# mobvoi/lstm_ctc

Measured on AMD Instinct MI355X. Metric: acoustic frames/sec (whole node), 5xBiLSTM-1024 CTC, higher is better.
Workload: dtype f32

## Files before the change

### include/lstm_ctc_hip.h

```cpp
#ifndef LSTM_CTC_HIP_H
#define LSTM_CTC_HIP_H

#include <stddef.h>
#include <stdint.h>

#ifdef __cplusplus
extern "C" {
#endif

#define LC_OK 0
#define LC_EINVAL (-1)
#define LC_ELAUNCH (-2)
#define LC_EWORKSPACE (-3)

typedef void *lc_stream_t;

const char *lc_last_error(void);
int lc_version(void);

#define LC_OPTION_UNSET (-0x7fffffffL - 1)
int lc_set_option(const char *name, long value);
int lc_get_option(const char *name, long *value);

size_t lc_ctc_workspace_bytes(int T, int B, int V, int max_label_len);
// ... 109 lines not shown
size_t lc_optimizer_workspace_bytes(size_t n);

size_t lc_colsum_workspace_bytes(int N);
int lc_colsum(const float *x, int rows, int N, int ldx, float *out, int accumulate, void *workspace,
              size_t workspace_bytes, lc_stream_t stream);
int lc_transpose(const float *in, int rows, int cols, float *out, lc_stream_t stream);

int lc_label_smoothing(const float *logits, int rows, int V, const float *log_q, float weight,
                       double *loss_acc, float *dlogits, lc_stream_t stream);

int lc_posteriors(const float *logits, int rows, int V, float smooth, int apply_softmax,
                  int apply_log, const float *log_prior, float *out, lc_stream_t stream);

size_t lc_bn_workspace_bytes(int C);
int lc_bn_moments(const float *x, int rows, int C, int ldx, float *mean, float *var, void *workspace,
                  size_t workspace_bytes, lc_stream_t stream);
int lc_bn_apply(const float *x, int rows, int C, int ldx, const float *mean, const float *var,
                const float *gamma, const float *beta, float eps, float *y, int ldy, lc_stream_t stream);
int lc_bn_bwd(const float *x, const float *dy, int rows, int C, int ldx, int lddy, const float *mean,
              const float *var, const float *gamma, float eps, int training, float *dx, int lddx,
              float *dgamma, float *dbeta, void *workspace, size_t workspace_bytes, lc_stream_t stream);
int lc_bn_update_moving(float *moving_mean, float *moving_var, const float *mean, const float *var, int C,
                        float momentum, lc_stream_t stream);
int lc_length_mask(float *x, int T, int B, int C, int ldx, const int *seq_len, lc_stream_t stream);

int lc_pack_rows(const float *x, int ldx, const int *rows, int Mp, int C, float *out, int ldo, lc_stream_t stream);
int lc_unpack_rows(const float *x, int ldx, const int *inverse, int rows, int C, float *out, int ldo, lc_stream_t stream);

void lc_debug_set_lstm_stamps(unsigned long long *buf);
int lc_debug_last_lstm_schedule(void);
void lc_debug_set_ctc_stamps(unsigned long long *buf);
int lc_debug_spin(int blocks, int microseconds, int lds_bytes, lc_stream_t stream);
int lc_debug_gemm_whole_round_row_tiles(int row_tiles, int col_tiles, int cus);

typedef struct {
    int64_t num_frames;
    int32_t dim;
    int32_t has_input, has_target;
    int64_t num_labels;
} lc_seqex_info_t;
int lc_tfrecord_inspect(const void *file, size_t nbytes, int verify_crc, lc_seqex_info_t *info);
int lc_tfrecord_decode(const void *file, size_t nbytes, int dim, int left_context, int right_context, int subsample,
                       float *x, size_t x_row_stride, int64_t max_rows, int64_t *labels, int64_t max_labels);
uint32_t lc_crc32c(const void *data, size_t nbytes);
typedef struct lc_batch_reader lc_batch_reader_t;
int lc_batch_open(const char *const *paths, int n, int verify_crc, int expect_dim, int nthreads,
                  lc_batch_reader_t **reader, int64_t *num_frames, int64_t *num_labels);
int lc_batch_decode(lc_batch_reader_t *reader, int left_context, int right_context, int subsample, float *x,
                    size_t utt_stride, size_t row_stride, int64_t max_rows, int64_t *labels, size_t label_stride,
                    int64_t max_labels, int64_t pad_label, int nthreads);
void lc_batch_close(lc_batch_reader_t *reader);

#ifdef __cplusplus
}
#endif
#endif
```

### lstm_ctc_amd/_lib.py

```python
import ctypes
import os

_HERE = os.path.dirname(os.path.abspath(__file__))
LIB_PATH = os.path.join(_HERE, "liblstm_ctc_hip.so")

c_int, c_float, c_void_p, c_size_t = ctypes.c_int, ctypes.c_float, ctypes.c_void_p, ctypes.c_size_t
c_u32 = ctypes.c_uint32

SIGNATURES = {
    "lc_last_error": (ctypes.c_char_p, []),
    "lc_version": (c_int, []),
    "lc_set_option": (c_int, [ctypes.c_char_p, ctypes.c_long]),
    "lc_get_option": (c_int, [ctypes.c_char_p, ctypes.POINTER(ctypes.c_long)]),
    "lc_ctc_workspace_bytes": (c_size_t, [c_int, c_int, c_int, c_int]),
    "lc_ctc_loss": (c_int, [c_void_p, c_int, c_int, c_int, c_void_p, c_void_p, c_void_p, c_int, c_void_p,
                            c_void_p, c_void_p, c_size_t, c_void_p]),
    "lc_ctc_greedy": (c_int, [c_void_p, c_int, c_int, c_int, c_void_p, c_void_p, c_void_p, c_void_p, c_void_p]),
    "lc_edit_distance_host": (c_int, [c_void_p, c_int, c_void_p, c_void_p, c_void_p, c_int, c_void_p]),
    "lc_gemm_workspace_bytes": (c_size_t, [c_int, c_int, c_int]),
    "lc_gemm_f32": (c_int, [c_int, c_int, c_int, c_int, c_int, c_float, c_void_p, c_int, c_void_p, c_int,
                            c_float, c_void_p, c_int, c_void_p, c_void_p, c_size_t, c_void_p]),
    "lc_gemm_bf16": (c_int, [c_int, c_int, c_int, c_int, c_int, c_float, c_void_p, c_int, c_void_p, c_int,
                             c_float, c_void_p, c_int, c_void_p, c_void_p, c_size_t, c_void_p]),
    "lc_bn_workspace_bytes": (c_size_t, [c_int]),
# ... 21 lines not shown
                                  c_void_p, c_void_p, ctypes.c_size_t, c_void_p]),
    "lc_gemm_next_epilogue": (c_int, [c_void_p]),
    "lc_gemm_bf16_nn": (c_int, [c_int, c_int, c_int, c_float, c_void_p, c_int, c_void_p, c_int, c_float, c_void_p, c_int,
                                c_void_p, c_void_p, c_size_t, c_void_p]),
    "lc_debug_set_lstm_stamps": (None, [c_void_p]),
    "lc_debug_set_ctc_stamps": (None, [c_void_p]),
    "lc_debug_spin": (c_int, [c_int, c_int, c_int, c_void_p]),
    "lc_length_mask": (c_int, [c_void_p, c_int, c_int, c_int, c_int, c_void_p, c_void_p]),
    "lc_pack_rows": (c_int, [c_void_p, c_int, c_void_p, c_int, c_int, c_void_p, c_int, c_void_p]),
    "lc_unpack_rows": (c_int, [c_void_p, c_int, c_void_p, c_int, c_int, c_void_p, c_int, c_void_p]),
    "lc_lstm_fwd_workspace_bytes": (c_size_t, [c_int, c_int, c_int]),
    "lc_lstm_fwd": (c_int, [c_void_p, c_int, c_void_p, c_int, c_int, c_int, c_float, c_void_p, c_size_t, c_void_p]),
    "lc_lstm_fwd_bf16": (c_int, [c_void_p, c_int, c_void_p, c_int, c_int, c_int, c_float, c_void_p, c_size_t, c_void_p]),
    "lc_lstm_fwd_x3": (c_int, [c_void_p, c_int, c_void_p, c_int, c_int, c_int, c_float, c_void_p, c_size_t, c_void_p]),
    "lc_lstm_bwd_x3": (c_int, [c_void_p, c_int, c_void_p, c_int, c_int, c_int, c_void_p, c_size_t, c_void_p]),
    "lc_lstm_bwd_workspace_bytes": (c_size_t, [c_int, c_int, c_int]),
    "lc_lstm_bwd_bf16": (c_int, [c_void_p, c_int, c_void_p, c_int, c_int, c_int, c_void_p, c_size_t, c_void_p]),
    "lc_lstm_bwd": (c_int, [c_void_p, c_int, c_void_p, c_int, c_int, c_int, c_void_p, c_size_t, c_void_p]),
    "lc_dropout_scale": (c_int, [c_void_p, c_int, c_int, c_int, c_float, c_u32, c_u32, c_void_p, c_int, c_int,
                                 c_void_p]),
    "lc_dropout_scale_bf16": (c_int, [c_void_p, c_int, c_int, c_int, c_float, c_u32, c_u32, c_void_p, c_int, c_int,
                                      c_void_p, c_int, c_void_p]),
    "lc_moe_combine_fwd": (c_int, [c_void_p, c_void_p, c_int, c_int, c_int, c_float, c_float, c_u32, c_void_p,
                                   c_void_p, c_void_p]),
    "lc_moe_combine_bwd": (c_int, [c_void_p, c_void_p, c_void_p, c_int, c_int, c_int, c_float, c_float, c_u32,
                                   c_void_p, c_void_p]),
    "lc_optimizer_workspace_bytes": (c_size_t, [c_size_t]),
    "lc_optimizer_step": (c_int, [c_void_p, c_void_p, c_size_t, c_size_t, c_float, c_float, c_int, c_float,
                                  c_int, c_void_p, c_void_p, c_void_p, c_void_p, c_size_t, c_void_p]),
    "lc_colsum_workspace_bytes": (c_size_t, [c_int]),
    "lc_colsum": (c_int, [c_void_p, c_int, c_int, c_int, c_void_p, c_int, c_void_p, c_size_t, c_void_p]),
    "lc_debug_last_lstm_schedule": (c_int, []),
    "lc_debug_gemm_whole_round_row_tiles": (c_int, [c_int, c_int, c_int]),
    "lc_transpose": (c_int, [c_void_p, c_int, c_int, c_void_p, c_void_p]),
    "lc_label_smoothing": (c_int, [c_void_p, c_int, c_int, c_void_p, c_float, c_void_p, c_void_p, c_void_p]),
    "lc_tfrecord_inspect": (c_int, [c_void_p, c_size_t, c_int, c_void_p]),
    "lc_tfrecord_decode": (c_int, [c_void_p, c_size_t, c_int, c_int, c_int, c_int, c_void_p, c_size_t, ctypes.c_int64,
                                   c_void_p, ctypes.c_int64]),
    "lc_crc32c": (c_u32, [c_void_p, c_size_t]),
    "lc_batch_open": (c_int, [c_void_p, c_int, c_int, c_int, c_int, c_void_p, c_void_p, c_void_p]),
    "lc_batch_decode": (c_int, [c_void_p, c_int, c_int, c_int, c_void_p, c_size_t, c_size_t, ctypes.c_int64, c_void_p,
                                c_size_t, ctypes.c_int64, ctypes.c_int64, c_int]),
    "lc_batch_close": (None, [c_void_p]),
    "lc_posteriors": (c_int, [c_void_p, c_int, c_int, c_float, c_int, c_int, c_void_p, c_void_p, c_void_p]),
}


class GemmEpilogue(ctypes.Structure):
    _fields_ = [("keep", ctypes.c_float), ("seed", ctypes.c_uint32), ("stream0", ctypes.c_uint32),
                ("drop_width", ctypes.c_int), ("c_bf16", ctypes.c_void_p), ("ldc_bf16", ctypes.c_int),
                ("shadow_only", ctypes.c_int)]


class SeqExInfo(ctypes.Structure):
    _fields_ = [("num_frames", ctypes.c_int64), ("dim", ctypes.c_int32), ("has_input", ctypes.c_int32),
                ("has_target", ctypes.c_int32), ("num_labels", ctypes.c_int64)]


class LstmFwdDir(ctypes.Structure):
    _fields_ = [("zx", c_void_p), ("R", c_void_p), ("w_f", c_void_p), ("w_i", c_void_p), ("w_o", c_void_p),
                ("cs", c_void_p), ("hs", c_void_p), ("reverse", c_int), ("hs_bf16", c_void_p), ("shadow_only", c_int)]


class LstmBwdDir(ctypes.Structure):
    _fields_ = [("gates", c_void_p), ("RT", c_void_p), ("w_f", c_void_p), ("w_i", c_void_p), ("w_o", c_void_p),
                ("cs", c_void_p), ("dh", c_void_p), ("dpeep", c_void_p), ("dbias", c_void_p), ("reverse", c_int),
# ... 39 lines not shown
```

### lstm_ctc_amd/csrc/common.h

```cpp
#pragma once
#include <hip/hip_runtime.h>
#include <stdint.h>
#include <stdio.h>
#include <stdarg.h>
#include "../../include/lstm_ctc_hip.h"

#define LC_WAVE 64

void lc_set_error(const char *fmt, ...);
enum { LC_OPT_LSTM_PERSISTENT = 0, LC_OPT_LSTM_SPIN_LIMIT, LC_OPT_GEMM_F32_BIG, LC_OPT_GEMM_BF16_BIG, LC_OPT_CTC_LSE2,
       LC_OPT_GEMM_BF16_PERSIST, LC_OPT_GEMM_TAIL };
long lc_option(int opt, long dflt);

#define LC_CHECK_ARG(cond, ...)                                   \
    do {                                                          \
        if (!(cond)) { lc_set_error(__VA_ARGS__); return LC_EINVAL; } \
    } while (0)

#define LC_CHECK_LAUNCH(what)                                                        \
    do {                                                                             \
        hipError_t e_ = hipGetLastError();                                           \
        if (e_ != hipSuccess) {                                                      \
            lc_set_error("%s: %s", what, hipGetErrorString(e_));                     \
            return LC_ELAUNCH;                                                       \
        }                                                                            \
    } while (0)

static inline int lc_cdiv(long long a, long long b) { return (int)((a + b - 1) / b); }

__host__ __device__ inline uint32_t lc_fmix32(uint32_t h)
{
    h ^= h >> 16; h *= 0x85EBCA6Bu; h ^= h >> 13; h *= 0xC2B2AE35u; h ^= h >> 16;
    return h;
}
__host__ __device__ inline float lc_dropout_factor(uint32_t seed, uint32_t stream, uint64_t idx,
                                                   float keep, float inv_keep)
{
    uint32_t h = (seed * 0x9E3779B1u) ^ (stream * 0x85EBCA77u + 0x165667B1u);
    uint32_t v = lc_fmix32((uint32_t)idx ^ h);
    v = lc_fmix32(v ^ ((uint32_t)(idx >> 32) + 0x27D4EB2Fu));
    float u = (float)(v >> 8) * (1.0f / 16777216.0f);
    return u < keep ? inv_keep : 0.0f;
}

// ... 47 lines not shown
```

### lstm_ctc_amd/csrc/error.cpp

```cpp
#include <limits.h>
#include <stdarg.h>
#include <stdio.h>
#include <stdlib.h>
#include <string.h>
#include "../../include/lstm_ctc_hip.h"

static thread_local char g_err[512] = "";

void lc_set_error(const char *fmt, ...)
{
    va_list ap;
    va_start(ap, fmt);
    vsnprintf(g_err, sizeof(g_err), fmt, ap);
    va_end(ap);
}

extern "C" const char *lc_last_error(void) { return g_err; }
extern "C" int lc_version(void) { return 2; }

static const char *const g_opt_name[] = {"lstm_persistent", "lstm_spin_limit", "gemm_f32_big", "gemm_bf16_big", "ctc_lse2",
                                         "gemm_bf16_persist", "gemm_tail"};
static const char *const g_opt_env[] = {"LC_LSTM_PERSISTENT", "LC_LSTM_SPIN_LIMIT", "LC_GEMM_F32_BIG",
                                        "LC_GEMM_BF16_BIG", "LC_CTC_LSE2", "LC_GEMM_BF16_PERSIST",
                                        "LC_GEMM_TAIL"};
enum { N_OPTS = sizeof(g_opt_name) / sizeof(g_opt_name[0]) };
static thread_local long g_opt_val[N_OPTS];
static thread_local bool g_opt_set[N_OPTS];

long lc_option(int opt, long dflt)
{
    if (opt < 0 || opt >= N_OPTS) return dflt;
    if (g_opt_set[opt]) return g_opt_val[opt];
    const char *env = getenv(g_opt_env[opt]);
    return env ? atol(env) : dflt;
}
static int opt_index(const char *name)
{
    for (int i = 0; name && i < N_OPTS; ++i)
        if (strcmp(name, g_opt_name[i]) == 0) return i;
    return -1;
}
extern "C" int lc_set_option(const char *name, long value)
{
    const int i = opt_index(name);
    if (i < 0) { lc_set_error("lc_set_option: unknown option '%s'", name ? name : "(null)"); return LC_EINVAL; }
    g_opt_set[i] = value != LC_OPTION_UNSET;
    g_opt_val[i] = value;
    return LC_OK;
}
extern "C" int lc_get_option(const char *name, long *value)
{
    const int i = opt_index(name);
    if (i < 0) { lc_set_error("lc_get_option: unknown option '%s'", name ? name : "(null)"); return LC_EINVAL; }
    const long v = lc_option(i, LC_OPTION_UNSET);
    if (value) *value = v;
    return LC_OK;
}
// ... 1 lines not shown
```

### lstm_ctc_amd/csrc/gemm.hip

```cpp
#include "common.h"
#include "gemm_epi.h"
#include <algorithm>

typedef float f32x16 __attribute__((ext_vector_type(16)));
typedef int i32x4 __attribute__((ext_vector_type(4)));
typedef float f32x4v __attribute__((ext_vector_type(4)));
__device__ f32x4v lc_raw_buffer_load_f32x4(i32x4 rsrc, int voffset, int soffset, int aux) __asm("llvm.amdgcn.raw.buffer.load.v4f32");
__device__ i32x4 lc_raw_buffer_load_i32x4(i32x4 rsrc, int voffset, int soffset, int aux) __asm("llvm.amdgcn.raw.buffer.load.v4i32");

namespace {

#ifndef LC_GEMM_BK
#define LC_GEMM_BK 16
#endif
#ifndef LC_GEMM_GROUP_M
#define LC_GEMM_GROUP_M 8
#endif
constexpr int BM = 128, BN = 128, BK = LC_GEMM_BK, NT = 256;

template <bool KMAJOR, bool FAST, int I>
__device__ __forceinline__ float4 tile_load1(const float *__restrict__ src, int ld, int c0, int cmax, int k0,
                                             int kmax, bool vec_ok)
{
    const int f = threadIdx.x + NT * I;
// ... 530 lines not shown
        const unsigned short *bs = Bs0 + (CUR) * 128 * SP + (wn * 64 + lr) * SP + lk * 8;                   \
        bf16x8 a0 = *reinterpret_cast<const bf16x8 *>(as), a1 = *reinterpret_cast<const bf16x8 *>(as + 32 * SP); \
        bf16x8 b0 = *reinterpret_cast<const bf16x8 *>(bs), b1 = *reinterpret_cast<const bf16x8 *>(bs + 32 * SP); \
        _Pragma("unroll") for (int q = 0; q < SBK / 16; ++q) {                                              \
            bf16x8 na0 = a0, na1 = a1, nb0 = b0, nb1 = b1;                                                  \
            if (q + 1 < SBK / 16) {                                                                         \
                na0 = *reinterpret_cast<const bf16x8 *>(as + (q + 1) * 16);                                 \
                na1 = *reinterpret_cast<const bf16x8 *>(as + 32 * SP + (q + 1) * 16);                       \
                nb0 = *reinterpret_cast<const bf16x8 *>(bs + (q + 1) * 16);                                 \
                nb1 = *reinterpret_cast<const bf16x8 *>(bs + 32 * SP + (q + 1) * 16);                       \
            }                                                                                               \
            acc[0][0] = __builtin_amdgcn_mfma_f32_32x32x16_bf16(a0, b0, acc[0][0], 0, 0, 0);                \
            acc[0][1] = __builtin_amdgcn_mfma_f32_32x32x16_bf16(a0, b1, acc[0][1], 0, 0, 0);                \
            acc[1][0] = __builtin_amdgcn_mfma_f32_32x32x16_bf16(a1, b0, acc[1][0], 0, 0, 0);                \
            acc[1][1] = __builtin_amdgcn_mfma_f32_32x32x16_bf16(a1, b1, acc[1][1], 0, 0, 0);                \
            a0 = na0; a1 = na1; b0 = nb0; b1 = nb1;                                                         \
        }                                                                                                   \
        stile_store(As0 + ((CUR) ^ 1) * 128 * SP, SA);                                                      \
        stile_store(Bs0 + ((CUR) ^ 1) * 128 * SP, SB);                                                      \
        __syncthreads();                                                                                    \
    }
    int kt = 0;
    for (; kt + 2 <= nk; kt += 2) {
        LC_SGEMM_STEP(kt, 0, ra0, rb0, ra1, rb1)
        LC_SGEMM_STEP(kt + 1, 1, ra1, rb1, ra0, rb0)
    }
    if (kt < nk) LC_SGEMM_STEP(kt, 0, ra0, rb0, ra1, rb1)
#undef LC_SGEMM_STEP
    gemm_epilogue<FAST>(p, acc, m0, n0, wm, wn, lr, lk);
}

constexpr int GBM = 256, GBN = 256, GBK = 64, GNT = 512;
constexpr int G_OPERAND_BYTES = 256 * GBK * 2;
__device__ __forceinline__ void gemm_tile_order_big(int M, int N, int &bm, int &bn, int bid = blockIdx.x)
{
    const int nbm = M / GBM, nbn = N / GBN;
    const int nwg = nbm * nbn;
    {
        const int q = nwg / 8, rr = nwg % 8, xcd = bid % 8, idx = bid / 8;
        bid = (xcd < rr ? xcd * (q + 1) : rr * (q + 1) + (xcd - rr) * q) + idx;
    }
    constexpr int GROUP_M = 4;
    const int gsz = GROUP_M * nbn;
    const int first_m = (bid / gsz) * GROUP_M;
    const int gm = min(nbm - first_m, GROUP_M);
    bm = first_m + (bid % gsz) % gm;
    bn = (bid % gsz) / gm;
}

typedef short s16x4 __attribute__((ext_vector_type(4)));
typedef int i32x2 __attribute__((ext_vector_type(2)));
template <int OFF>
__device__ __forceinline__ void tr16_pair(unsigned lds_addr, i32x2 &lo, i32x2 &hi)
{
    asm volatile("ds_read_b64_tr_b16 %0, %2 offset:%3\n\tds_read_b64_tr_b16 %1, %2 offset:%4"
                 : "=&v"(lo), "=&v"(hi)
                 : "v"(lds_addr), "n"(OFF), "n"(OFF + 2048));
}
typedef int i32x4g __attribute__((ext_vector_type(4)));
template <int OFF>
__device__ __forceinline__ void lds_read128(unsigned lds_addr, i32x4g &v)
{
    asm volatile("ds_read_b128 %0, %1 offset:%2" : "=&v"(v) : "v"(lds_addr), "n"(OFF));
}
__device__ __forceinline__ bf16x8 frag_cast(i32x4g v)
{
    union { i32x4g i; bf16x8 b; } u;
    u.i = v;
    return u.b;
}
__device__ __forceinline__ bf16x8 tr16_join(i32x2 lo, i32x2 hi)
{
    union { i32x2 h[2]; bf16x8 v; } u;
    u.h[0] = lo; u.h[1] = hi;
    return u.v;
}
template <bool ACOL, bool BCOL, bool PERSIST = false, bool SEG2 = false>
__global__ __launch_bounds__(GNT, 1) void gemm_bf16g_kernel(SGemmArgs sp)
{
    __shared__ __attribute__((aligned(1024))) unsigned char lds[4 * G_OPERAND_BYTES];
// ... 356 lines not shown
#pragma unroll
        for (int i = 0; i < 4; ++i)
#pragma unroll
            for (int j = 0; j < 2; ++j) {
                const int col = n0 + wn * 64 + j * 32 + lr;
#pragma unroll
                for (int r = 0; r < 16; ++r) {
                    const int row = m0 + wm * 128 + i * 32 + (r & 3) + 8 * (r >> 2) + 4 * lk;
                    S[(size_t)row * p.slab_ld + col] = acc[i][j][r];
                }
            }
        return;
    }
#pragma unroll
    for (int i = 0; i < 4; ++i)
#pragma unroll
        for (int j = 0; j < 2; ++j) {
            const int col = n0 + wn * 64 + j * 32 + lr;
            const float bv = p.bias ? p.bias[col] : 0.f;
            unsigned est;
            int ecm;
            epi_column(p.epi, col, est, ecm);
#pragma unroll
            for (int r = 0; r < 16; ++r) {
                const int row = m0 + wm * 128 + i * 32 + (r & 3) + 8 * (r >> 2) + 4 * lk;
                float *c = p.C + (size_t)row * p.ldc + col;
                float v = p.alpha * acc[i][j][r] + bv;
                if (p.beta != 0.f) v += p.beta * *c;
                epi_store(p.epi, c, v, row, col, est, ecm);
            }
        }
}

__global__ __launch_bounds__(256) void cast_bf16_kernel(const float *__restrict__ x, int rows, int C, int ldx,
                                                        unsigned short *__restrict__ nat, int ldnat,
                                                        unsigned short *__restrict__ tr, int ldtr)
{
    __shared__ unsigned short tile[64][66];
    const int r0 = blockIdx.y * 64, c0 = blockIdx.x * 64;
    const int tx = threadIdx.x & 63, ty = threadIdx.x >> 6;
    for (int i = ty; i < 64; i += 4) {
        const int r = r0 + i, c = c0 + tx;
        unsigned short v = 0;
        if (r < rows && c < C) {
            v = __builtin_bit_cast(unsigned short, (__bf16)x[(size_t)r * ldx + c]);
            if (nat) nat[(size_t)r * ldnat + c] = v;
        }
        tile[i][tx] = v;
    }
    if (!tr) return;
    __syncthreads();
    for (int i = ty; i < 64; i += 4) {
        const int c = c0 + i, r = r0 + tx;
        if (c < C && r < rows) tr[(size_t)c * ldtr + r] = tile[tx][i];
    }
}

__device__ __forceinline__ unsigned cast_pack2(float lo, float hi)
{
    return (unsigned)__builtin_bit_cast(unsigned short, (__bf16)lo) |
           ((unsigned)__builtin_bit_cast(unsigned short, (__bf16)hi) << 16);
}
template <bool NAT, bool TR>
__global__ __launch_bounds__(256) void cast_bf16_vec_kernel(const float *__restrict__ x, int ldx,
                                                            unsigned short *__restrict__ nat, int ldnat,
                                                            unsigned short *__restrict__ tr, int ldtr)
// ... 91 lines not shown

static int lc_num_cus()
{
    static int cached[16] = {0};
    int dev = 0;
    if (hipGetDevice(&dev) != hipSuccess || dev < 0 || dev >= 16) return 256;
    if (cached[dev] == 0) {
        int n = 0;
        if (hipDeviceGetAttribute(&n, hipDeviceAttributeMultiprocessorCount, dev) != hipSuccess || n <= 0) n = 256;
        cached[dev] = n;
    }
    return cached[dev];
}
static int gemm_whole_round_row_tiles(int row_tiles, int col_tiles, int cus_override = 0)
{
    const int cus = cus_override > 0 ? cus_override : lc_num_cus();
    if (lc_option(LC_OPT_GEMM_TAIL, 0) == 0 || row_tiles <= 1 || col_tiles <= 0) return row_tiles;
    const long long tiles = (long long)row_tiles * col_tiles;
    if (tiles % cus == 0 || tiles < 2ll * cus) return row_tiles;
    double best_t = (double)((tiles + cus - 1) / cus) - 0.05;
    int best = row_tiles;
    for (int keep = row_tiles - 1, it = 0; keep >= 1 && it < 512; --keep, ++it) {
        const long long big = (long long)keep * col_tiles, rem = big % cus;
        if (big < cus) break;
        if (rem != 0 && rem * 100 < (long long)cus * 97) continue;
        const double t = (double)((big + cus - 1) / cus) + (double)(row_tiles - keep) * col_tiles * 4 * 0.275 / cus + 0.1;
        if (t < best_t) { best_t = t; best = keep; }
    }
    return best;
}
extern "C" int lc_debug_gemm_whole_round_row_tiles(int row_tiles, int col_tiles, int cus)
{
    return gemm_whole_round_row_tiles(row_tiles, col_tiles, cus);
}
static bool bf16g_persist_ok(long long tiles, int nsl, int K)
{
    const int cus = lc_num_cus();
    return lc_option(LC_OPT_GEMM_BF16_PERSIST, 0) != 0 && nsl <= 1 && K % (2 * GBK) == 0 && cus % 8 == 0 && tiles > cus;
}

static const EpiArgs EPI_NONE = {1.f, 1.f, 0u, 0u, 1, nullptr, 0, 0, 0};
static thread_local EpiArgs g_epi_next = EPI_NONE;
EpiArgs lc_epi_take()
{
    const EpiArgs e = g_epi_next;
    g_epi_next = EPI_NONE;
    return e;
}
static EpiArgs epi_take() { return lc_epi_take(); }
extern "C" int lc_gemm_next_epilogue(const lc_gemm_epilogue_t *e)
{
    if (!e) { g_epi_next = EPI_NONE; return LC_OK; }
    LC_CHECK_ARG(e->keep > 0.f && e->keep <= 1.f && (e->keep >= 1.f || e->drop_width > 0),
                 "lc_gemm_next_epilogue: keep must be in (0, 1] and drop_width > 0");
    LC_CHECK_ARG(!e->c_bf16 || e->ldc_bf16 > 0, "lc_gemm_next_epilogue: ldc_bf16 must be positive");
    EpiArgs a = EPI_NONE;
    a.keep = e->keep; a.inv_keep = 1.0f / e->keep; a.seed = e->seed; a.stream0 = e->stream0;
    a.P = e->keep < 1.f ? e->drop_width : 1;
    a.c16 = (unsigned short *)e->c_bf16; a.ldc16 = e->ldc_bf16;
    LC_CHECK_ARG(!e->shadow_only || e->c_bf16, "lc_gemm_next_epilogue: shadow_only needs c_bf16");
    a.skip_c = e->shadow_only ? 1 : 0;
    g_epi_next = a;
    return LC_OK;
}

extern "C" size_t lc_gemm_workspace_bytes(int M, int N, int K)
// ... 27 lines not shown
                       int lda, const float *B, int ldb, float beta, float *C, int ldc, const float *bias,
                       void *workspace, size_t workspace_bytes, lc_stream_t stream)
{
    const EpiArgs epi = epi_take();
    LC_CHECK_ARG(A && B && C, "%s: null pointer", who);
    LC_CHECK_ARG(M >= 0 && N >= 0 && K >= 0, "%s: negative dimension", who);
    if (M == 0 || N == 0) return LC_OK;
    LC_CHECK_ARG(lda >= (ta ? M : K) && ldb >= (tb ? K : N) && ldc >= N, "%s: leading dimension too small", who);
    hipStream_t s = (hipStream_t)stream;
    const int bk = bf16 ? HBK : BK;
    if (epi_active(epi)) { workspace = nullptr; workspace_bytes = 0; }
    GemmArgs p;
    p.epi = epi;
    p.A2 = p.B2 = nullptr; p.k1 = 0;
    p.M = M; p.N = N; p.K = K; p.alpha = alpha; p.beta = beta;
    p.A = A; p.lda = lda; p.B = B; p.ldb = ldb; p.C = C; p.ldc = ldc; p.bias = bias;
    p.vecA = aligned16(A) && (lda % 4 == 0);
    p.vecB = aligned16(B) && (ldb % 4 == 0);
    LC_CHECK_ARG((long long)lc_cdiv(M, BM) * lc_cdiv(N, BN) < (1ll << 31), "%s: grid too large", who);
    const int big_mode = (int)lc_option(LC_OPT_GEMM_F32_BIG, 1);
    if (!bf16 && big_mode != 0 && p.vecA && p.vecB && K >= FGBK && K % FGBK == 0) {
        int Mi = M / GBM * GBM;
        const int Ni = N / GBN * GBN;
        const bool exact = Mi == M && Ni == N;
        int nb = exact ? pick_splitk_big(M, N, K, FGBK) : 1;
        if (nb > 1 && (!workspace || workspace_bytes < (size_t)nb * M * N * sizeof(float))) nb = 1;
        if (nb <= 1) Mi = gemm_whole_round_row_tiles(Mi / GBM, Ni / GBN) * GBM;
        const long long tiles = (long long)(Mi / GBM) * (Ni / GBN);
        const long long spanA = ta ? (long long)K * lda * 4 + 4ll * GBM : (long long)(GBM - 1) * lda * 4 + 4ll * K;
        const long long spanB = tb ? (long long)(GBN - 1) * ldb * 4 + 4ll * K : (long long)K * ldb * 4 + 4ll * GBN;
        const long long wgs = tiles * (nb > 1 ? nb : 1), rounds = (wgs + 255) / 256;
        const bool fills = wgs >= 128 && wgs * 10 >= rounds * 256 * 9;
        if (tiles > 0 && (fills || big_mode == 2) && spanA < 0x7fffffffll && spanB < 0x7fffffffll) {
            GemmArgs q = p;
            q.M = Mi; q.N = Ni;
            q.kchunk = nb > 1 ? lc_cdiv(lc_cdiv(K, nb), FGBK) * FGBK : K;
            if (nb > 1) nb = lc_cdiv(K, q.kchunk);
            q.slab = nb > 1 ? (float *)workspace : nullptr;
            q.slab_slice = (size_t)M * N;
            q.slab_ld = N;
            const dim3 grid((unsigned)tiles, 1, (unsigned)(nb > 1 ? nb : 1)), block(GNT);
            if (ta && !tb) hipLaunchKernelGGL((gemm_f32g_kernel<true, true>), grid, block, 0, s, q);
            else if (ta) hipLaunchKernelGGL((gemm_f32g_kernel<true, false>), grid, block, 0, s, q);
            else if (!tb) hipLaunchKernelGGL((gemm_f32g_kernel<false, true>), grid, block, 0, s, q);
            else hipLaunchKernelGGL((gemm_f32g_kernel<false, false>), grid, block, 0, s, q);
            p.kchunk = K > 0 ? K : 1; p.slab = nullptr; p.slab_slice = 0; p.slab_ld = N;
            if (Ni < N) {
                q = p;
                q.N = N - Ni;
                q.B = tb ? B + (size_t)Ni * ldb : B + Ni;
                q.C = C + Ni;
                q.epi = epi_block(p.epi, 0, Ni);
                q.bias = bias ? bias + Ni : nullptr;
                q.vecB = aligned16(q.B) && (ldb % 4 == 0);
                gemm_launch_part(false, false, ta, tb, q, 1, s);
            }
            if (Mi < M) {
                q = p;
                q.M = M - Mi; q.N = Ni;
                q.A = ta ? A + Mi : A + (size_t)Mi * lda;
                q.C = C + (size_t)Mi * ldc;
                q.epi = epi_block(p.epi, Mi, 0);
                q.vecA = aligned16(q.A) && (lda % 4 == 0);
                const bool fast = q.M % BM == 0 && q.N % BN == 0 && K % BK == 0 && q.vecA && q.vecB;
                gemm_launch_part(false, fast, ta, tb, q, 1, s);
            }
            LC_CHECK_LAUNCH(who);
            if (nb > 1) {
                const size_t quads = (size_t)M * N / 4;
                int g = (int)((quads + 255) / 256);
                if (g > 2048) g = 2048;
                hipLaunchKernelGGL(splitk_reduce_kernel, dim3(g), dim3(256), 0, s, (float *)workspace, nb, M, N, alpha, beta, C, ldc, bias);
                LC_CHECK_LAUNCH("splitk_reduce");
            }
            return LC_OK;
        }
    }
    int nsl = pick_splitk(M, N, K);
// ... 42 lines not shown
        if (g > 2048) g = 2048;
        hipLaunchKernelGGL(splitk_reduce_kernel, dim3(g), dim3(256), 0, s, p.slab, nsl, M, N, alpha, beta, C, ldc, bias);
        LC_CHECK_LAUNCH("splitk_reduce");
    }
    return LC_OK;
}

extern "C" int lc_gemm_f32(int ta, int tb, int M, int N, int K, float alpha, const float *A, int lda,
                           const float *B, int ldb, float beta, float *C, int ldc, const float *bias,
                           void *workspace, size_t workspace_bytes, lc_stream_t stream)
{
    return gemm_launch(false, "lc_gemm_f32", ta, tb, M, N, K, alpha, A, lda, B, ldb, beta, C, ldc, bias, workspace,
                       workspace_bytes, stream);
}

extern "C" int lc_gemm_f32_nt2(int M, int N, int K1, int K2, float alpha, const float *A1, const float *A2, int lda,
                               const float *B1, const float *B2, int ldb, float beta, float *C, int ldc, const float *bias,
                               lc_stream_t stream)
{
    const EpiArgs epi = epi_take();
    const char *who = "lc_gemm_f32_nt2";
    LC_CHECK_ARG(A1 && A2 && B1 && B2 && C, "%s: null pointer", who);
    LC_CHECK_ARG(M >= 0 && N >= 0 && K1 > 0 && K2 > 0, "%s: bad dimension", who);
    if (M == 0 || N == 0) return LC_OK;
    LC_CHECK_ARG(lda >= std::max(K1, K2) && ldb >= std::max(K1, K2) && ldc >= N, "%s: leading dimension too small", who);
    hipStream_t s = (hipStream_t)stream;
    auto sequence = [&](int m, int n, const float *a1, const float *a2, const float *b1, const float *b2, float *c,
                        const float *bi, const EpiArgs &e) -> int {
        int rc = gemm_launch(false, who, 0, 1, m, n, K1, alpha, a1, lda, b1, ldb, beta, c, ldc, bi, nullptr, 0, stream);
        if (rc != LC_OK) return rc;
        g_epi_next = e;
        return gemm_launch(false, who, 0, 1, m, n, K2, alpha, a2, lda, b2, ldb, 1.f, c, ldc, nullptr, nullptr, 0, stream);
    };
    const int Mi = M / GBM * GBM, Ni = N / GBN * GBN;
    const long long tiles = (long long)(Mi / GBM) * (Ni / GBN), rounds = (tiles + 255) / 256;
    const int big_mode = (int)lc_option(LC_OPT_GEMM_F32_BIG, 1);
    const bool vec = aligned16(A1) && aligned16(A2) && aligned16(B1) && aligned16(B2) && lda % 4 == 0 && ldb % 4 == 0;
    const bool fills = tiles >= 128 && tiles * 10 >= rounds * 256 * 9;
    const long long span = (long long)(GBM - 1) * std::max(lda, ldb) * 4 + 4ll * std::max(K1, K2);
    if (!(big_mode != 0 && vec && tiles > 0 && (fills || big_mode == 2) && K1 % FGBK == 0 && K2 % FGBK == 0 &&
          span < 0x7fffffffll))
        return sequence(M, N, A1, A2, B1, B2, C, bias, epi);
    GemmArgs q;
    q.epi = epi;
    q.M = Mi; q.N = Ni; q.K = K1 + K2; q.alpha = alpha; q.beta = beta;
    q.A = A1; q.lda = lda; q.B = B1; q.ldb = ldb; q.C = C; q.ldc = ldc; q.bias = bias;
    q.vecA = q.vecB = 1;
    q.kchunk = K1 + K2; q.slab = nullptr; q.slab_slice = 0; q.slab_ld = N;
    q.A2 = A2; q.B2 = B2; q.k1 = K1;
    hipLaunchKernelGGL((gemm_f32g_kernel<false, false, true>), dim3((unsigned)tiles, 1, 1), dim3(GNT), 0, s, q);
    LC_CHECK_LAUNCH(who);
    if (Ni < N) {
        const int rc = sequence(M, N - Ni, A1, A2, B1 + (size_t)Ni * ldb, B2 + (size_t)Ni * ldb, C + Ni,
                                bias ? bias + Ni : nullptr, epi_block(epi, 0, Ni));
        if (rc != LC_OK) return rc;
    }
    if (Mi < M) {
        const int rc = sequence(M - Mi, Ni, A1 + (size_t)Mi * lda, A2 + (size_t)Mi * lda, B1, B2, C + (size_t)Mi * ldc, bias,
                                epi_block(epi, Mi, 0));
        if (rc != LC_OK) return rc;
    }
    return LC_OK;
}
extern "C" int lc_gemm_bf16(int ta, int tb, int M, int N, int K, float alpha, const float *A, int lda,
                            const float *B, int ldb, float beta, float *C, int ldc, const float *bias,
                            void *workspace, size_t workspace_bytes, lc_stream_t stream)
{
    return gemm_launch(true, "lc_gemm_bf16", ta, tb, M, N, K, alpha, A, lda, B, ldb, beta, C, ldc, bias, workspace,
                       workspace_bytes, stream);
}

extern "C" int lc_cast_bf16(const float *x, int rows, int C, int ldx, uint16_t *nat, int ldnat, uint16_t *tr, int ldtr,
                            lc_stream_t stream)
{
    LC_CHECK_ARG(x && (nat || tr) && rows >= 0 && C > 0 && ldx >= C, "lc_cast_bf16: bad argument");
    LC_CHECK_ARG((!nat || ldnat >= C) && (!tr || ldtr >= rows), "lc_cast_bf16: leading dimension too small");
    if (rows == 0) return LC_OK;
    if (rows % 64 == 0 && C % 64 == 0 && ldx % 4 == 0 && aligned16(x) && (!nat || (ldnat % 4 == 0 && (((uintptr_t)nat) & 7) == 0)) &&
        (!tr || (ldtr % 8 == 0 && aligned16(tr)))) {
        const dim3 grid(C / 64, rows / 64), block(256);
        hipStream_t s = (hipStream_t)stream;
        if (nat && tr) hipLaunchKernelGGL((cast_bf16_vec_kernel<true, true>), grid, block, 0, s, x, ldx, nat, ldnat, tr, ldtr);
        else if (nat) hipLaunchKernelGGL((cast_bf16_vec_kernel<true, false>), grid, block, 0, s, x, ldx, nat, ldnat, tr, ldtr);
// ... 247 lines not shown
```

Measured before the change: 189,000.

## Balance last GEMM wave with variable-height row tiles for partial rounds

Adds an 'even' plan for the f32 GEMM that keeps some whole 256x256 tiles and re-splits the remaining rows (plus any 32-row tail) into shorter tiles of h*32 rows. These run in a second kernel sized so the last wave fills the CUs instead of leaving many idle in a partial round. A cost model chooses how many whole row tiles to keep. This adds a second launch and shorter tiles with less reuse per block, and it is on by default unless the tail option is set.

```diff
diff --git a/include/lstm_ctc_hip.h b/include/lstm_ctc_hip.h
--- a/include/lstm_ctc_hip.h
+++ b/include/lstm_ctc_hip.h
@@ -165,6 +165,7 @@
 void lc_debug_set_ctc_stamps(unsigned long long *buf);
 int lc_debug_spin(int blocks, int microseconds, int lds_bytes, lc_stream_t stream);
 int lc_debug_gemm_whole_round_row_tiles(int row_tiles, int col_tiles, int cus);
+int lc_debug_gemm_even_plan(int row_tiles, int col_tiles, int extra_blocks, int cus, int *out);
 
 typedef struct {
     int64_t num_frames;
diff --git a/lstm_ctc_amd/_lib.py b/lstm_ctc_amd/_lib.py
--- a/lstm_ctc_amd/_lib.py
+++ b/lstm_ctc_amd/_lib.py
@@ -77,6 +77,7 @@
     "lc_colsum": (c_int, [c_void_p, c_int, c_int, c_int, c_void_p, c_int, c_void_p, c_size_t, c_void_p]),
     "lc_debug_last_lstm_schedule": (c_int, []),
     "lc_debug_gemm_whole_round_row_tiles": (c_int, [c_int, c_int, c_int]),
+    "lc_debug_gemm_even_plan": (c_int, [c_int, c_int, c_int, c_int, c_void_p]),
     "lc_transpose": (c_int, [c_void_p, c_int, c_int, c_void_p, c_void_p]),
     "lc_label_smoothing": (c_int, [c_void_p, c_int, c_int, c_void_p, c_float, c_void_p, c_void_p, c_void_p]),
     "lc_tfrecord_inspect": (c_int, [c_void_p, c_size_t, c_int, c_void_p]),
diff --git a/lstm_ctc_amd/csrc/common.h b/lstm_ctc_amd/csrc/common.h
--- a/lstm_ctc_amd/csrc/common.h
+++ b/lstm_ctc_amd/csrc/common.h
@@ -9,7 +9,7 @@
 
 void lc_set_error(const char *fmt, ...);
 enum { LC_OPT_LSTM_PERSISTENT = 0, LC_OPT_LSTM_SPIN_LIMIT, LC_OPT_GEMM_F32_BIG, LC_OPT_GEMM_BF16_BIG, LC_OPT_CTC_LSE2,
-       LC_OPT_GEMM_BF16_PERSIST, LC_OPT_GEMM_TAIL };
+       LC_OPT_GEMM_BF16_PERSIST, LC_OPT_GEMM_TAIL, LC_OPT_GEMM_EVEN };
 long lc_option(int opt, long dflt);
 
 #define LC_CHECK_ARG(cond, ...)                                   \
diff --git a/lstm_ctc_amd/csrc/error.cpp b/lstm_ctc_amd/csrc/error.cpp
--- a/lstm_ctc_amd/csrc/error.cpp
+++ b/lstm_ctc_amd/csrc/error.cpp
@@ -19,10 +19,10 @@
 extern "C" int lc_version(void) { return 2; }
 
 static const char *const g_opt_name[] = {"lstm_persistent", "lstm_spin_limit", "gemm_f32_big", "gemm_bf16_big", "ctc_lse2",
-                                         "gemm_bf16_persist", "gemm_tail"};
+                                         "gemm_bf16_persist", "gemm_tail", "gemm_even"};
 static const char *const g_opt_env[] = {"LC_LSTM_PERSISTENT", "LC_LSTM_SPIN_LIMIT", "LC_GEMM_F32_BIG",
                                         "LC_GEMM_BF16_BIG", "LC_CTC_LSE2", "LC_GEMM_BF16_PERSIST",
-                                        "LC_GEMM_TAIL"};
+                                        "LC_GEMM_TAIL", "LC_GEMM_EVEN"};
 enum { N_OPTS = sizeof(g_opt_name) / sizeof(g_opt_name[0]) };
 static thread_local long g_opt_val[N_OPTS];
 static thread_local bool g_opt_set[N_OPTS];
diff --git a/lstm_ctc_amd/csrc/gemm.hip b/lstm_ctc_amd/csrc/gemm.hip
--- a/lstm_ctc_amd/csrc/gemm.hip
+++ b/lstm_ctc_amd/csrc/gemm.hip
@@ -586,9 +586,8 @@
 
 constexpr int GBM = 256, GBN = 256, GBK = 64, GNT = 512;
 constexpr int G_OPERAND_BYTES = 256 * GBK * 2;
-__device__ __forceinline__ void gemm_tile_order_big(int M, int N, int &bm, int &bn, int bid = blockIdx.x)
-{
-    const int nbm = M / GBM, nbn = N / GBN;
+__device__ __forceinline__ void gemm_tile_order_tiles(int nbm, int nbn, int &bm, int &bn, int bid = blockIdx.x)
+{
     const int nwg = nbm * nbn;
     {
         const int q = nwg / 8, rr = nwg % 8, xcd = bid % 8, idx = bid / 8;
@@ -600,6 +599,10 @@
     const int gm = min(nbm - first_m, GROUP_M);
     bm = first_m + (bid % gsz) % gm;
     bn = (bid % gsz) / gm;
+}
+__device__ __forceinline__ void gemm_tile_order_big(int M, int N, int &bm, int &bn, int bid = blockIdx.x)
+{
+    gemm_tile_order_tiles(M / GBM, N / GBN, bm, bn, bid);
 }
 
 typedef short s16x4 __attribute__((ext_vector_type(4)));
@@ -1022,6 +1025,128 @@
         }
 }
 
+struct EvenArgs { int nst, nh; };
+template <int R, bool BCOL, bool SEG2 = false>
+__global__ __launch_bounds__(GNT, 1) void gemm_f32e_kernel(GemmArgs p, EvenArgs e)
+{
+    static_assert(R >= 1 && R <= 8, "32 .. 256 rows");
+    static_assert(!SEG2 || !BCOL, "two operand pairs: NT form");
+    __shared__ __attribute__((aligned(1024))) unsigned char lds[4 * 256 * FGBK * 4];
+    constexpr int OPB = 256 * FGBK * 4;
+    int st, bn;
+    gemm_tile_order_tiles(e.nst, p.N / GBN, st, bn);
+    const int rl = st < e.nh ? R : R - 1;
+    const int m0 = 32 * (st < e.nh ? st * R : e.nh * R + (st - e.nh) * (R - 1)), n0 = bn * GBN;
+    const int lane = threadIdx.x & 63, wave = __builtin_amdgcn_readfirstlane(threadIdx.x >> 6);
+    const int nk = p.K / FGBK;
+    const float *abase = p.A + (size_t)m0 * p.lda;
+    const float *bbase = BCOL ? p.B + n0 : p.B + (size_t)n0 * p.ldb;
+    const __amdgpu_buffer_rsrc_t ra = __builtin_amdgcn_make_buffer_rsrc((void *)abase, 0, 0x7fffffff, 0x00020000);
+    const __amdgpu_buffer_rsrc_t rb = __builtin_amdgcn_make_buffer_rsrc((void *)bbase, 0, 0x7fffffff, 0x00020000);
+    const int nk1 = SEG2 ? p.k1 / FGBK : nk;
+    const __amdgpu_buffer_rsrc_t ra2 = SEG2 ? __builtin_amdgcn_make_buffer_rsrc((void *)(p.A2 + (size_t)m0 * p.lda), 0,
+                                                                                0x7fffffff, 0x00020000) : ra;
+    const __amdgpu_buffer_rsrc_t rb2 = SEG2 ? __builtin_amdgcn_make_buffer_rsrc((void *)(p.B2 + (size_t)n0 * p.ldb), 0,
+                                                                                0x7fffffff, 0x00020000) : rb;
+    constexpr int NPA = (4 * R + 7) / 8;
+    int voa[4], vob[4];
+#pragma unroll
+    for (int i = 0; i < NPA; ++i) {
+        const int row = (i * 8 + wave) * 8 + (lane >> 3);
+        voa[i] = (row * p.lda + ((lane & 7) ^ ((row >> 1) & 7)) * 4) * 4;
+    }
+#pragma unroll
+    for (int i = 0; i < 4; ++i) {
+        const int piece = wave * 4 + i;
+        if (BCOL) vob[i] = (piece * p.ldb + 4 * lane) * 4;
+        else { const int row = piece * 8 + (lane >> 3); vob[i] = (row * p.ldb + ((lane & 7) ^ ((row >> 1) & 7)) * 4) * 4; }
+    }
+    const int ka = FGBK * 4, kb = BCOL ? FGBK * p.ldb * 4 : FGBK * 4;
+    const int npa = 4 * rl;
+#define LC_EFILL_FROM(RA, RB, KT, BUF)                                                                                 \
+    {                                                                                                                  \
+        _Pragma("unroll") for (int i = 0; i < NPA; ++i)                                                                \
+            if (i * 8 + wave < npa)                                                                                    \
+                __builtin_amdgcn_raw_ptr_buffer_load_lds(RA, lds + (BUF) * 2 * OPB + (i * 8 + wave) * 1024, 16, voa[i], \
+                                                         (KT) * ka, 0, 0);                                             \
+        _Pragma("unroll") for (int i = 0; i < 4; ++i)                                                                  \
+            __builtin_amdgcn_raw_ptr_buffer_load_lds(RB, lds + ((BUF) * 2 + 1) * OPB + (wave * 4 + i) * 1024, 16,       \
+                                                     vob[i], (KT) * kb, 0, 0);                                         \
+    }
+#define LC_EFILL(KT, BUF)                                                                                              \
+    {                                                                                                                  \
+        const int kt_ = (KT);                                                                                          \
+        if (SEG2 && kt_ >= nk1) LC_EFILL_FROM(ra2, rb2, kt_ - nk1, BUF) else LC_EFILL_FROM(ra, rb, kt_, BUF)           \
+    }
+    f32x16 acc[R];
+#pragma unroll
+    for (int i = 0; i < R; ++i)
+#pragma unroll
+        for (int r = 0; r < 16; ++r) acc[i][r] = 0.f;
+    const int lr = lane & 31, lk = lane >> 5;
+    const int fl = (lr >> 1) & 7;
+    int soq[4];
+#pragma unroll
+    for (int q = 0; q < 4; ++q) soq[q] = ((2 * q + lk) ^ fl) * 16;
+    const int arow = lr * 128;
+    const int brow = BCOL ? (4 * lk * 256 + wave * 32 + lr) * 4 : (wave * 32 + lr) * 128;
+#define LC_ECOMPUTE(BUF)                                                                                               \
+    {                                                                                                                  \
+        const unsigned char *as = lds + (BUF) * 2 * OPB + arow;                                                        \
+        const unsigned char *bs = lds + ((BUF) * 2 + 1) * OPB + brow;                                                  \
+        _Pragma("unroll") for (int q = 0; q < 4; ++q) {                                                                \
+            float a[R][4], b[4];                                                                                       \
+            _Pragma("unroll") for (int i = 0; i < R; ++i) {                                                            \
+                const f32x4v v = *reinterpret_cast<const f32x4v *>(as + i * 4096 + soq[q]);                            \
+                a[i][0] = v.x; a[i][1] = v.y; a[i][2] = v.z; a[i][3] = v.w;                                            \
+            }                                                                                                          \
+            if (BCOL) {                                                                                                \
+                _Pragma("unroll") for (int t = 0; t < 4; ++t)                                                          \
+                    b[t] = *reinterpret_cast<const float *>(bs + (8 * q + t) * 256 * 4);                               \
+            } else {                                                                                                   \
+                const f32x4v v = *reinterpret_cast<const f32x4v *>(bs + soq[q]);                                       \
+                b[0] = v.x; b[1] = v.y; b[2] = v.z; b[3] = v.w;                                                        \
+            }                                                                                                          \
+            _Pragma("unroll") for (int t = 0; t < 4; ++t)                                                              \
+                _Pragma("unroll") for (int i = 0; i < R; ++i)                                                          \
+                    acc[i] = __builtin_amdgcn_mfma_f32_32x32x2f32(a[i][t], b[t], acc[i], 0, 0, 0);                     \
+        }                                                                                                              \
+    }
+    LC_EFILL(0, 0)
+    __syncthreads();
+    int kt = 0;
+    for (; kt + 2 <= nk; kt += 2) {
+        LC_EFILL(min(kt + 1, nk - 1), 1)
+        LC_ECOMPUTE(0)
+        __syncthreads();
+        LC_EFILL(min(kt + 2, nk - 1), 0)
+        LC_ECOMPUTE(1)
+        __syncthreads();
+    }
+    if (kt < nk) LC_ECOMPUTE(0)
+#undef LC_EFILL
+#undef LC_EFILL_FROM
+#undef LC_ECOMPUTE
+    const int col = n0 + wave * 32 + lr;
+    const float bv = p.bias ? p.bias[col] : 0.f;
+    unsigned est;
+    int ecm;
+    epi_column(p.epi, col, est, ecm);
+#pragma unroll
+    for (int i = 0; i < R; ++i) {
+        if (i < rl) {
+#pragma unroll
+            for (int r = 0; r < 16; ++r) {
+                const int row = m0 + i * 32 + (r & 3) + 8 * (r >> 2) + 4 * lk;
+                float *c = p.C + (size_t)row * p.ldc + col;
+                float v = p.alpha * acc[i][r] + bv;
+                if (p.beta != 0.f) v += p.beta * *c;
+                epi_store(p.epi, c, v, row, col, est, ecm);
+            }
+        }
+    }
+}
+
 __global__ __launch_bounds__(256) void cast_bf16_kernel(const float *__restrict__ x, int rows, int C, int ldx,
                                                         unsigned short *__restrict__ nat, int ldnat,
                                                         unsigned short *__restrict__ tr, int ldtr)
@@ -1179,6 +1304,49 @@
 extern "C" int lc_debug_gemm_whole_round_row_tiles(int row_tiles, int col_tiles, int cus)
 {
     return gemm_whole_round_row_tiles(row_tiles, col_tiles, cus);
+}
+struct EvenPlan { int whole, h, nh, nh1; };
+static EvenPlan gemm_even_plan(int row_tiles, int col_tiles, int extra_blocks, int cus_override = 0)
+{
+    const int cus = cus_override > 0 ? cus_override : lc_num_cus();
+    EvenPlan best = {row_tiles, 0, 0, 0};
+    if (row_tiles < 1 || col_tiles < 1 || extra_blocks < 0 || extra_blocks > 7 || col_tiles > cus) return best;
+    const long long tiles = (long long)row_tiles * col_tiles, rounds = (tiles + cus - 1) / cus;
+    if (rounds < 2 || (tiles % cus == 0 && extra_blocks == 0)) return best;
+    const int S = cus / col_tiles;
+    double best_t = (double)rounds + (extra_blocks > 0 ? 0.375 : 0.0);
+    for (int keep = extra_blocks > 0 ? row_tiles : row_tiles - 1; keep >= 1; --keep) {
+        const long long blocks = (long long)(row_tiles - keep) * 8 + extra_blocks, big = (long long)keep * col_tiles;
+        if (blocks > 8ll * S || big < cus) break;
+        const int h = (int)((blocks + S - 1) / S);
+        const double t = (double)((big + cus - 1) / cus) + h / 8.0 + 0.05;
+        if (t < best_t - 1e-9) {
+            best_t = t;
+            const int nh = (int)(blocks - (long long)(h - 1) * S);
+            best = {keep, h, nh, h > 1 ? S - nh : 0};
+        }
+    }
+    return best;
+}
+extern "C" int lc_debug_gemm_even_plan(int row_tiles, int col_tiles, int extra_blocks, int cus, int *out)
+{
+    const EvenPlan e = gemm_even_plan(row_tiles, col_tiles, extra_blocks, cus);
+    if (out) { out[0] = e.whole; out[1] = e.h; out[2] = e.nh; out[3] = e.nh1; }
+    return e.h > 0 ? 1 : 0;
+}
+static bool gemm_even_enabled() { return lc_option(LC_OPT_GEMM_EVEN, 1) != 0 && lc_option(LC_OPT_GEMM_TAIL, 0) == 0; }
+static void gemm_even_launch(int form, const EvenPlan &e, const GemmArgs &q, hipStream_t s)
+{
+    const EvenArgs ea = {e.nh + e.nh1, e.nh};
+    const dim3 grid((unsigned)(ea.nst * (q.N / GBN))), block(GNT);
+#define LC_EVEN(R)                                                                                              \
+    case R:                                                                                                     \
+        if (form == 0) hipLaunchKernelGGL((gemm_f32e_kernel<R, true>), grid, block, 0, s, q, ea);               \
+        else if (form == 1) hipLaunchKernelGGL((gemm_f32e_kernel<R, false>), grid, block, 0, s, q, ea);         \
+        else hipLaunchKernelGGL((gemm_f32e_kernel<R, false, true>), grid, block, 0, s, q, ea);                  \
+        break;
+    switch (e.h) { LC_EVEN(1) LC_EVEN(2) LC_EVEN(3) LC_EVEN(4) LC_EVEN(5) LC_EVEN(6) LC_EVEN(7) LC_EVEN(8) default: break; }
+#undef LC_EVEN
 }
 static bool bf16g_persist_ok(long long tiles, int nsl, int K)
 {
@@ -1272,6 +1440,11 @@
         const long long wgs = tiles * (nb > 1 ? nb : 1), rounds = (wgs + 255) / 256;
         const bool fills = wgs >= 128 && wgs * 10 >= rounds * 256 * 9;
         if (tiles > 0 && (fills || big_mode == 2) && spanA < 0x7fffffffll && spanB < 0x7fffffffll) {
+            EvenPlan even = {Mi / GBM, 0, 0, 0};
+            if (nb <= 1 && !ta && gemm_even_enabled())
+                even = gemm_even_plan(Mi / GBM, Ni / GBN, (M - Mi) % 32 == 0 ? (M - Mi) / 32 : 0);
+            const int Me = even.h > 0 ? 32 * (even.nh * even.h + even.nh1 * (even.h - 1)) : 0;
+            if (even.h > 0) Mi = even.whole * GBM;
             GemmArgs q = p;
             q.M = Mi; q.N = Ni;
             q.kchunk = nb > 1 ? lc_cdiv(lc_cdiv(K, nb), FGBK) * FGBK : K;
@@ -1279,11 +1452,19 @@
             q.slab = nb > 1 ? (float *)workspace : nullptr;
             q.slab_slice = (size_t)M * N;
             q.slab_ld = N;
-            const dim3 grid((unsigned)tiles, 1, (unsigned)(nb > 1 ? nb : 1)), block(GNT);
+            const dim3 grid((unsigned)((long long)(Mi / GBM) * (Ni / GBN)), 1, (unsigned)(nb > 1 ? nb : 1)), block(GNT);
             if (ta && !tb) hipLaunchKernelGGL((gemm_f32g_kernel<true, true>), grid, block, 0, s, q);
             else if (ta) hipLaunchKernelGGL((gemm_f32g_kernel<true, false>), grid, block, 0, s, q);
             else if (!tb) hipLaunchKernelGGL((gemm_f32g_kernel<false, true>), grid, block, 0, s, q);
             else hipLaunchKernelGGL((gemm_f32g_kernel<false, false>), grid, block, 0, s, q);
+            if (even.h > 0) {
+                q.M = Me;
+                q.A = A + (size_t)Mi * lda;
+                q.C = C + (size_t)Mi * ldc;
+                q.epi = epi_block(p.epi, Mi, 0);
+                gemm_even_launch(tb ? 1 : 0, even, q, s);
+                Mi += Me;
+            }
             p.kchunk = K > 0 ? K : 1; p.slab = nullptr; p.slab_slice = 0; p.slab_ld = N;
             if (Ni < N) {
                 q = p;
@@ -1392,7 +1573,8 @@
         g_epi_next = e;
         return gemm_launch(false, who, 0, 1, m, n, K2, alpha, a2, lda, b2, ldb, 1.f, c, ldc, nullptr, nullptr, 0, stream);
     };
-    const int Mi = M / GBM * GBM, Ni = N / GBN * GBN;
+    int Mi = M / GBM * GBM;
+    const int Ni = N / GBN * GBN;
     const long long tiles = (long long)(Mi / GBM) * (Ni / GBN), rounds = (tiles + 255) / 256;
     const int big_mode = (int)lc_option(LC_OPT_GEMM_F32_BIG, 1);
     const bool vec = aligned16(A1) && aligned16(A2) && aligned16(B1) && aligned16(B2) && lda % 4 == 0 && ldb % 4 == 0;
@@ -1408,7 +1590,19 @@
     q.vecA = q.vecB = 1;
     q.kchunk = K1 + K2; q.slab = nullptr; q.slab_slice = 0; q.slab_ld = N;
     q.A2 = A2; q.B2 = B2; q.k1 = K1;
-    hipLaunchKernelGGL((gemm_f32g_kernel<false, false, true>), dim3((unsigned)tiles, 1, 1), dim3(GNT), 0, s, q);
+    EvenPlan even = {Mi / GBM, 0, 0, 0};
+    if (gemm_even_enabled()) even = gemm_even_plan(Mi / GBM, Ni / GBN, (M - Mi) % 32 == 0 ? (M - Mi) / 32 : 0);
+    if (even.h > 0) { Mi = even.whole * GBM; q.M = Mi; }
+    hipLaunchKernelGGL((gemm_f32g_kernel<false, false, true>), dim3((unsigned)((long long)(Mi / GBM) * (Ni / GBN)), 1, 1),
+                       dim3(GNT), 0, s, q);
+    if (even.h > 0) {
+        q.M = 32 * (even.nh * even.h + even.nh1 * (even.h - 1));
+        q.A = A1 + (size_t)Mi * lda; q.A2 = A2 + (size_t)Mi * lda;
+        q.C = C + (size_t)Mi * ldc;
+        q.epi = epi_block(epi, Mi, 0);
+        gemm_even_launch(2, even, q, s);
+        Mi += q.M;
+    }
     LC_CHECK_LAUNCH(who);
     if (Ni < N) {
         const int rc = sequence(M, N - Ni, A1, A2, B1 + (size_t)Ni * ldb, B2 + (size_t)Ni * ldb, C + Ni,
```

New measurement: 190,100 (median of 6 runs). No clear change (+0.6%).
